# cmbant/getdist

Measured on AMD Instinct MI355X. Metric: 2D KDE densities/sec (triangle, 50 params, 1e+07 samples), higher is better.
Workload: dtype f64

## Files before the change

### getdist_amd/csrc/binning.hip

```cpp
#include "ctx.hpp"

#include <array>
#include <map>

#define LDS_HIST_BYTES (128 * 1024)

struct BinDiv {
    double binmin, width, rcp;
};
__device__ __forceinline__ BinDiv make_bindiv(double binmin, double width) {
    BinDiv d;
    d.binmin = binmin, d.width = width;
    const unsigned long long mant = (unsigned long long)__double_as_longlong(width) & 0xFFFFFFFFFFFFFull;
    d.rcp = (mant == 0xFFFFFFFFFFFFFull) ? 0.0 : 1.0 / width;
    return d;
}
__device__ __forceinline__ double bin_quotient(double x, const BinDiv& d) {
    const double n = x - d.binmin;
    double q = n * d.rcp;
    double r = fma(-q, d.width, n);
    q = fma(r, d.rcp, q);
    r = fma(-q, d.width, n);
    q = fma(r, d.rcp, q);
    if (!(fabs(q) < 1e300) || d.rcp == 0.0) q = n / d.width;
    return q;
}
__device__ __forceinline__ int bin_round(double x, const BinDiv& d) {
    return (int)(bin_quotient(x, d) + 0.5);
}
__device__ __forceinline__ int bin_trunc(double x, const BinDiv& d) {
    return (int)bin_quotient(x, d);
}

template <bool HAS_W>
__global__ void __launch_bounds__(256) k_hist1d(const double* __restrict__ cols, int64_t ld,
                                                const int32_t* __restrict__ colidx, const double* __restrict__ w,
                                                int64_t N, const double* __restrict__ binmin,
                                                const double* __restrict__ width, int F, double* __restrict__ part) {
    extern __shared__ double sh[];
    const int c = blockIdx.y;
    const double* x = cols + (int64_t)colidx[c] * ld;
    const BinDiv bd = make_bindiv(binmin[c], width[c]);
    for (int i = threadIdx.x; i < 4 * F; i += 256) sh[i] = 0;
    __syncthreads();
    double* mine = sh + (threadIdx.x >> 6) * F;
    const int64_t gtid = (int64_t)blockIdx.x * 256 + threadIdx.x, gsz = (int64_t)gridDim.x * 256;
    const int64_t Ne = N & ~(int64_t)1;
    for (int64_t i = 2 * gtid; i < Ne; i += 2 * gsz) {
        const double2 xv = *reinterpret_cast<const double2*>(x + i);
        double2 wv = make_double2(1.0, 1.0);
        if (HAS_W) wv = *reinterpret_cast<const double2*>(w + i);
        const int i0 = bin_round(xv.x, bd), i1 = bin_round(xv.y, bd);
        if ((unsigned)i0 < (unsigned)F) atomicAdd(&mine[i0], wv.x);
        if ((unsigned)i1 < (unsigned)F) atomicAdd(&mine[i1], wv.y);
    }
    if (gtid == 0 && Ne < N) {
        const int i0 = bin_round(x[Ne], bd);
        if ((unsigned)i0 < (unsigned)F) atomicAdd(&mine[i0], HAS_W ? w[Ne] : 1.0);
    }
    __syncthreads();
    double* p = part + ((int64_t)c * gridDim.x + blockIdx.x) * F;
    for (int i = threadIdx.x; i < F; i += 256) p[i] = (sh[i] + sh[F + i]) + (sh[2 * F + i] + sh[3 * F + i]);
}

__global__ void k_hist1d_reduce(const double* __restrict__ part, int nblk, int F, double* __restrict__ out) {
    const int f = blockIdx.x * blockDim.x + threadIdx.x;
    if (f >= F) return;
    const double* p = part + (int64_t)blockIdx.y * nblk * F + f;
    double s = 0;
    for (int b = 0; b < nblk; ++b) s += p[(int64_t)b * F];
    out[(int64_t)blockIdx.y * F + f] = s;
}

template <bool ROUND, typename T>
__global__ void k_bin_indices(const double* __restrict__ x, int64_t N, double binmin, double width, int F,
                              T* __restrict__ idx, unsigned long long* __restrict__ n_bad) {
    unsigned long long bad = 0;
    const BinDiv bd = make_bindiv(binmin, width);
    for (int64_t i = (int64_t)blockIdx.x * blockDim.x + threadIdx.x; i < N; i += (int64_t)gridDim.x * blockDim.x) {
        const int v = ROUND ? bin_round(x[i], bd) : bin_trunc(x[i], bd);
        idx[i] = (T)v;
        bad += ((unsigned)v >= (unsigned)F);
    }
// ... 598 lines not shown
    int64_t R = (ctx->N + nblk - 1) / nblk;
    if (R < 131072) R = 131072;
    R = (R + 4095) / 4096 * 4096;
    nblk = (int)((ctx->N + R - 1) / R);
    if (nblk < 1) nblk = 1;
    S.nblk = nblk, S.R = R, S.cap = (int)(R / 8);
    if (const char* e = getenv("GDHIP_BUCKET_LIST_CAP"))
        if (atoi(e) > 0 && atoi(e) < S.cap) S.cap = atoi(e);
    return S;
}
static int64_t bucket_route_bytes(const gd_ctx* ctx, const BucketRoute& R) {
    if (R.recs.empty()) return 0;
    const int nc = (int)R.recs.size();
    const BucketShape S = bucket_shape(ctx, nc);
    return ((int64_t)nc * sizeof(PrebinColB) + 255) / 256 * 256 + ((int64_t)nc * R.nbmax * 2 + 255) / 256 * 256 +
           ((int64_t)nc * 8 + 255) / 256 * 256 + ((int64_t)nc * S.nblk * 4 + 255) / 256 * 256 + (int64_t)nc * S.nblk * S.cap * 4 + 256;
}
template <bool OUT8>
static int bucket_route_launch(gd_ctx* ctx, const BucketRoute& R, char* base, int F, unsigned long long** bad_dev) {
    const int nc = (int)R.recs.size();
    const BucketShape S = bucket_shape(ctx, nc);
    int64_t off = 0;
    auto take = [&](int64_t bytes) {
        int64_t o = off;
        off += (bytes + 255) / 256 * 256;
        return o;
    };
    const int64_t o_recs = take((int64_t)nc * sizeof(PrebinColB)), o_lut = take((int64_t)nc * R.nbmax * 2), o_bad = take((int64_t)nc * 8),
                  o_cnt = take((int64_t)nc * S.nblk * 4), o_list = take((int64_t)nc * S.nblk * S.cap * 4);
    PrebinColB* d_recs = (PrebinColB*)(base + o_recs);
    unsigned short* d_lut = (unsigned short*)(base + o_lut);
    unsigned long long* d_bad = (unsigned long long*)(base + o_bad);
    int* d_cnt = (int*)(base + o_cnt);
    unsigned int* d_list = (unsigned int*)(base + o_list);
    GD_TRY(gd_h2d(ctx, d_recs, R.recs.data(), (size_t)nc * sizeof(PrebinColB)));
    GD_HIP(hipMemsetAsync(d_bad, 0, (size_t)nc * 8, ctx->stream));
    k_bucket_lut<<<dim3(R.nbmax / 256, nc), 256, 0, ctx->stream>>>(d_recs, F, R.nbmax, d_lut);
    GD_KERNEL_CHECK();
    const size_t lds = (size_t)R.nbmax * 2;
    GD_HIP(hipFuncSetAttribute((const void*)k_prebin_bq<OUT8>, hipFuncAttributeMaxDynamicSharedMemorySize, (int)lds));
    k_prebin_bq<OUT8><<<dim3(S.nblk, nc), 512, lds, ctx->stream>>>(d_recs, ctx->N, S.R, S.cap, R.nbmax, d_lut, d_list, d_cnt);
    GD_KERNEL_CHECK();
    k_prebin_fix<OUT8><<<dim3(S.nblk, nc), 256, 0, ctx->stream>>>(d_recs, ctx->N, S.R, S.cap, F, d_list, d_cnt, d_bad);
    GD_KERNEL_CHECK();
    *bad_dev = d_bad;
    return GD_OK;
}

#ifndef P16_UNROLL
#define P16_UNROLL 4
#endif
template <int MODE>
__global__ void __launch_bounds__(1024) k_hist2d_f64_p16(const Hist2DPair* __restrict__ pairs, int B, int64_t N, int F, int R,
                                                         int nstripes, int nchunks, int tile_major,
                                                         unsigned int* __restrict__ part, int* __restrict__ overflow) {
    extern __shared__ double sh_raw[];
    unsigned int* sh = reinterpret_cast<unsigned int*>(sh_raw);
    __shared__ double red[16];
    int pair, chunk, stripe;
    if (tile_major)
        decode_block_tiles(B, nstripes, nchunks, pair, chunk, stripe);
    else
        decode_block(nstripes, nchunks, pair, chunk, stripe);
    if (pair >= B) return;
    const Hist2DPair P = pairs[pair];
    const BinDiv bdx = make_bindiv(P.bx, P.wx), bdy = make_bindiv(P.by, P.wy);
    const int row0 = stripe * R;
    const int nwords = (R * F + 1) / 2;
    for (int i = threadIdx.x; i < nwords; i += 1024) sh[i] = 0;
    __syncthreads();
    int64_t per = (N + nchunks - 1) / nchunks;
    per = (per + 7) & ~(int64_t)7;
    const int64_t lo = (int64_t)chunk * per;
    int64_t hi = lo + per;
    if (hi > N) hi = N;
    if (hi < lo) hi = lo;
    unsigned int nacc = 0;
    auto visit = [&](double xv, double yv) {
        int cx, cy;
        if (MODE == 0) {
            cx = bin_round(xv, bdx), cy = bin_round(yv, bdy);
        } else {
            cx = bin_trunc(xv, bdx);
            cy = bin_trunc(P.r0 * xv + P.r1 * yv, bdy);
        }
        const unsigned r = (unsigned)cy - (unsigned)row0;
        if (r < (unsigned)R && (unsigned)cx < (unsigned)F && (unsigned)cy < (unsigned)F) {
            const unsigned a = r * (unsigned)F + (unsigned)cx;
            atomicAdd(&sh[a >> 1], 1u << ((a & 1u) * 16u));
            nacc += 1;
        }
    };
    const int64_t hi2 = lo + ((hi - lo) & ~(int64_t)1);
    int64_t i = lo + 2 * (int64_t)threadIdx.x;
    for (; i + (int64_t)(P16_UNROLL - 1) * 2 * 1024 < hi2; i += (int64_t)P16_UNROLL * 2 * 1024) {
        double2 xv[P16_UNROLL], yv[P16_UNROLL];
#pragma unroll
        for (int u = 0; u < P16_UNROLL; ++u) {
            xv[u] = gload_d2(P.x + i + (int64_t)u * 2 * 1024);
            yv[u] = gload_d2(P.y + i + (int64_t)u * 2 * 1024);
        }
#pragma unroll
        for (int u = 0; u < P16_UNROLL; ++u) {
            visit(xv[u].x, yv[u].x);
            visit(xv[u].y, yv[u].y);
        }
    }
    for (; i < hi2; i += 2 * 1024) {
        const double2 xv = gload_d2(P.x + i);
        const double2 yv = gload_d2(P.y + i);
        visit(xv.x, yv.x);
        visit(xv.y, yv.y);
    }
    if (threadIdx.x == 0 && hi2 < hi) visit(P.x[hi2], P.y[hi2]);
    __syncthreads();
    unsigned int* dst = part + (((int64_t)pair * nchunks + chunk) * nstripes + stripe) * (int64_t)nwords;
    unsigned int total = 0;
    for (int i = threadIdx.x; i < nwords; i += 1024) {
        const unsigned int v = sh[i];
        total += (v & 0xffffu) + (v >> 16);
        dst[i] = v;
    }
    const double t = block_sum((double)total, red), a = block_sum((double)nacc, red);
    if (threadIdx.x == 0 && t != a) atomicOr(&overflow[pair], 1);
}

__global__ void __launch_bounds__(1024) k_hist2d_u16_chunks(const Hist2DPair* __restrict__ pairs, int B, int64_t N, int F, int R,
                                                            int nstripes, int nchunks, unsigned int* __restrict__ part,
                                                            int* __restrict__ overflow) {
    extern __shared__ double sh_raw[];
    unsigned int* sh = reinterpret_cast<unsigned int*>(sh_raw);
    __shared__ double red[16];
    int pair, chunk, stripe;
    decode_block(nstripes, nchunks, pair, chunk, stripe);
    if (pair >= B) return;
    const Hist2DPair P = pairs[pair];
    const int row0 = stripe * R;
    const int nwords = (R * F + 1) / 2;
    for (int i = threadIdx.x; i < nwords; i += 1024) sh[i] = 0;
    __syncthreads();
    int64_t per = (N + nchunks - 1) / nchunks;
    per = (per + 7) & ~(int64_t)7;
    const int64_t lo = (int64_t)chunk * per;
    int64_t hi = lo + per;
    if (hi > N) hi = N;
    unsigned int nacc = 0;
    auto visit = [&](unsigned cx, unsigned cy) {
        const unsigned r = cy - (unsigned)row0;
        if (r < (unsigned)R && cx < (unsigned)F && cy < (unsigned)F) {
            const unsigned a = r * (unsigned)F + cx;
            atomicAdd(&sh[a >> 1], 1u << ((a & 1u) * 16u));
            nacc += 1;
        }
    };
    const int64_t hi8 = lo < hi ? lo + ((hi - lo) & ~(int64_t)7) : lo;
    auto visit8 = [&](const uint4& ax, const uint4& ay) {
        const unsigned xs[4] = {ax.x, ax.y, ax.z, ax.w}, ys[4] = {ay.x, ay.y, ay.z, ay.w};
#pragma unroll
        for (int q = 0; q < 4; ++q) {
            visit(xs[q] & 0xFFFFu, ys[q] & 0xFFFFu);
            visit(xs[q] >> 16, ys[q] >> 16);
        }
    };
    constexpr int DEPTH = 3;
    const int64_t nvec = (hi8 - lo) >> 3;
    const int64_t K = (nvec >> 10) / DEPTH * DEPTH;
    const uint4* gx = reinterpret_cast<const uint4*>(P.ix + lo);
    const uint4* gy = reinterpret_cast<const uint4*>(P.iy + lo);
    if (K > 0) {
        uint4 rx[DEPTH], ry[DEPTH];
#pragma unroll
        for (int d = 0; d < DEPTH; ++d) {
            rx[d] = gload_u4(gx + d * 1024 + threadIdx.x), ry[d] = gload_u4(gy + d * 1024 + threadIdx.x);
            __builtin_amdgcn_sched_barrier(0);
        }
        for (int64_t k = 0; k < K; k += DEPTH) {
            const int64_t kn = (k + DEPTH < K ? k + DEPTH : K - DEPTH) * 1024 + threadIdx.x;
#pragma unroll
            for (int d = 0; d < DEPTH; ++d) {
                visit8(rx[d], ry[d]);
                rx[d] = gload_u4(gx + kn + d * 1024), ry[d] = gload_u4(gy + kn + d * 1024);
                __builtin_amdgcn_sched_barrier(0);
            }
        }
    }
    for (int64_t u = K * 1024 + threadIdx.x; u < nvec; u += 1024) visit8(gload_u4(gx + u), gload_u4(gy + u));
    if (threadIdx.x == 0)
        for (int64_t i = hi8; i < hi; ++i) visit(P.ix[i], P.iy[i]);
    __syncthreads();
    unsigned int* dst = part + (((int64_t)pair * nchunks + chunk) * nstripes + stripe) * (int64_t)nwords;
    unsigned int total = 0;
    for (int i = threadIdx.x; i < nwords; i += 1024) {
        const unsigned int v = sh[i];
        total += (v & 0xffffu) + (v >> 16);
        dst[i] = v;
    }
    const double t = block_sum((double)total, red), a = block_sum((double)nacc, red);
    if (threadIdx.x == 0 && t != a) atomicOr(&overflow[pair], 1);
}

__global__ void __launch_bounds__(256) k_p16_reduce(const unsigned int* __restrict__ part, int F, int R, int nstripes, int nchunks,
                                                    double* __restrict__ hist_all) {
    const int pair = blockIdx.z, stripe = blockIdx.y;
    const int nwords = (R * F + 1) / 2;
    const int rows = min(R, F - stripe * R);
    const int wd = blockIdx.x * 256 + threadIdx.x;
    if (2 * wd >= rows * F) return;
    const int64_t step = (int64_t)nstripes * nwords;
    const unsigned int* p = part + ((int64_t)pair * nchunks * nstripes + stripe) * (int64_t)nwords + wd;
    unsigned int lo = 0, hi = 0;
    int c = 0;
    for (; c + 8 <= nchunks; c += 8) {
        unsigned int v[8];
#pragma unroll
        for (int q = 0; q < 8; ++q) v[q] = __builtin_nontemporal_load(p + (c + q) * step);
#pragma unroll
        for (int q = 0; q < 8; ++q) lo += v[q] & 0xffffu, hi += v[q] >> 16;
    }
    for (; c < nchunks; ++c) {
        const unsigned int v = p[c * step];
        lo += v & 0xffffu, hi += v >> 16;
    }
    double* hist = hist_all + (int64_t)pair * F * F + (int64_t)stripe * R * F;
    hist[2 * wd] = (double)lo;
    if (2 * wd + 1 < rows * F) hist[2 * wd + 1] = (double)hi;
}

__global__ void k_minmax_affine(const Hist2DPair* __restrict__ pairs, int64_t N, double* __restrict__ part) {
    __shared__ double red[16];
    const Hist2DPair P = pairs[blockIdx.y];
    double mn = INFINITY, mx = -INFINITY;
    const int64_t gtid = (int64_t)blockIdx.x * blockDim.x + threadIdx.x, gsz = (int64_t)gridDim.x * blockDim.x;
    const int64_t Ne = N & ~(int64_t)1;
    for (int64_t i = 2 * gtid; i < Ne; i += 2 * gsz) {
        const double2 xv = gload_d2(P.x + i);
        const double2 yv = gload_d2(P.y + i);
        const double p0 = P.r0 * xv.x + P.r1 * yv.x, p1 = P.r0 * xv.y + P.r1 * yv.y;
        mn = fmin(mn, fmin(p0, p1));
        mx = fmax(mx, fmax(p0, p1));
    }
    if (gtid == 0 && Ne < N) {
        const double p0 = P.r0 * P.x[Ne] + P.r1 * P.y[Ne];
        mn = fmin(mn, p0);
        mx = fmax(mx, p0);
    }
    const double r0 = block_min(mn, red), r1 = block_max(mx, red);
    if (threadIdx.x == 0) {
        double* p = part + ((int64_t)blockIdx.y * gridDim.x + blockIdx.x) * 2;
        p[0] = r0, p[1] = r1;
    }
}

#define MMG_COLS 8
#define MMG_PAIRS 16
struct MinmaxGroup {
    const double* col[MMG_COLS];
    double r0[MMG_PAIRS], r1[MMG_PAIRS];
    int a[MMG_PAIRS], b[MMG_PAIRS];
    int ncols, npairs;
};

__global__ void __launch_bounds__(256) k_minmax_affine_grouped(const MinmaxGroup* __restrict__ groups, int64_t N,
                                                               double* __restrict__ part) {
    __shared__ double2 slot[MMG_COLS][256];
    __shared__ double red[16];
    const MinmaxGroup& G = groups[blockIdx.y];
    const int ncols = G.ncols, npairs = G.npairs;
    double mn[MMG_PAIRS], mx[MMG_PAIRS];
#pragma unroll
    for (int p = 0; p < MMG_PAIRS; ++p) mn[p] = INFINITY, mx[p] = -INFINITY;
    const int64_t gtid = (int64_t)blockIdx.x * blockDim.x + threadIdx.x, gsz = (int64_t)gridDim.x * blockDim.x;
    const int64_t Ne = N & ~(int64_t)1;
    for (int64_t i = 2 * gtid; i < Ne; i += 2 * gsz) {
        double2 v[MMG_COLS];
#pragma unroll
        for (int c = 0; c < MMG_COLS; ++c) v[c] = gload_d2(G.col[min(c, ncols - 1)] + i);
        __builtin_amdgcn_sched_barrier(0);
#pragma unroll
        for (int c = 0; c < MMG_COLS; ++c) slot[c][threadIdx.x] = v[c];
#pragma unroll
        for (int p = 0; p < MMG_PAIRS; ++p)
            if (p < npairs) {
                const double2 xv = slot[G.a[p]][threadIdx.x], yv = slot[G.b[p]][threadIdx.x];
                const double p0 = G.r0[p] * xv.x + G.r1[p] * yv.x, p1 = G.r0[p] * xv.y + G.r1[p] * yv.y;
                mn[p] = fmin(mn[p], fmin(p0, p1));
                mx[p] = fmax(mx[p], fmax(p0, p1));
            }
    }
    if (gtid == 0 && Ne < N) {
#pragma unroll
        for (int p = 0; p < MMG_PAIRS; ++p)
            if (p < npairs) {
                const double p0 = G.r0[p] * G.col[G.a[p]][Ne] + G.r1[p] * G.col[G.b[p]][Ne];
                mn[p] = fmin(mn[p], p0);
                mx[p] = fmax(mx[p], p0);
            }
    }
    double* out = part + ((int64_t)blockIdx.y * gridDim.x + blockIdx.x) * MMG_PAIRS * 2;
#pragma unroll
    for (int p = 0; p < MMG_PAIRS; ++p)
        if (p < npairs) {
            const double r0 = block_min(mn[p], red), r1 = block_max(mx[p], red);
            if (threadIdx.x == 0) out[2 * p] = r0, out[2 * p + 1] = r1;
        }
}

static int pick_chunks(const gd_ctx* ctx, int64_t units, int64_t rows) {
    int best = 1;
    double best_cost = 1e30;
    for (int c = 1; c <= 16; ++c) {
        if ((int64_t)c * 65536 > rows && c > 1) break;
        const int64_t blocks = units * c;
        const double rounds = (double)((blocks + ctx->cu_count - 1) / ctx->cu_count);
        const double cost = rounds / c + 0.004 * c;
        if (cost < best_cost - 1e-12) best_cost = cost, best = c;
    }
    return best;
}

template <int MODE>
static int launch_hist2d(gd_ctx* ctx, int B, const std::vector<Hist2DPair>& hp, int F, double* d_hist, bool allow_p16 = true);

template <int MODE>
static int launch_hist2d_p16(gd_ctx* ctx, int B, const std::vector<Hist2DPair>& hp, int F, double* d_hist) {
    int R = LDS_HIST_BYTES / (F * 2);
    if (R > F) R = F;
    const int nstripes = (F + R - 1) / R;
    int nchunks = pick_chunks(ctx, (int64_t)B * nstripes, ctx->N);
    const int nwords = (R * F + 1) / 2;
    int tile_major = 0;
    if (B >= 16 && nstripes == 1 && ctx->N >= (1 << 20) && getenv("GDHIP_P16_TILE_MAJOR") != nullptr) {
        int64_t tiles = (ctx->N + 131071) / 131072;
        const int64_t cap = ((int64_t)3 << 30) / ((int64_t)B * nwords * 4);
        if (tiles > cap) tiles = cap;
        if (tiles > nchunks) nchunks = (int)tiles, tile_major = 1;
    }
    const int units = (B * nchunks + 7) / 8 * 8;
    const int64_t nblocks = (int64_t)units * nstripes;
    int64_t off = 0;
    auto take = [&](int64_t bytes) {
        int64_t o = off;
        off += (bytes + 255) / 256 * 256;
        return o;
    };
    const int64_t o_pairs = take((int64_t)B * sizeof(Hist2DPair)), o_flags = take((int64_t)B * 4),
                  o_part = take((int64_t)B * nchunks * nstripes * nwords * 4);
    char* base = (char*)gd_scratch2(ctx, off);
    if (!base) return GD_ERR_NOMEM;
    Hist2DPair* d_pairs = (Hist2DPair*)(base + o_pairs);
    int* d_flags = (int*)(base + o_flags);
    unsigned int* d_part = (unsigned int*)(base + o_part);
    GD_TRY(gd_h2d(ctx, d_pairs, hp.data(), (size_t)B * sizeof(Hist2DPair)));
    GD_HIP(hipMemsetAsync(d_flags, 0, (size_t)B * 4, ctx->stream));
    GD_HIP(hipFuncSetAttribute((const void*)k_hist2d_f64_p16<MODE>, hipFuncAttributeMaxDynamicSharedMemorySize, LDS_HIST_BYTES));
    k_hist2d_f64_p16<MODE><<<(unsigned)nblocks, 1024, (size_t)nwords * 4, ctx->stream>>>(d_pairs, B, ctx->N, F, R, nstripes,
                                                                                      nchunks, tile_major, d_part, d_flags);
    GD_KERNEL_CHECK();
    k_p16_reduce<<<dim3((unsigned)((nwords + 255) / 256), nstripes, B), 256, 0, ctx->stream>>>(d_part, F, R, nstripes, nchunks, d_hist);
    GD_KERNEL_CHECK();
    std::vector<int> hf((size_t)B);
    GD_TRY(gd_fetch(ctx, hf.data(), d_flags, (size_t)B * 4));
    GD_TRY(gd_stream_sync(ctx));
    std::vector<int> flagged;
    for (int b = 0; b < B; ++b)
        if (hf[b]) flagged.push_back(b);
    int rc = GD_OK;
    if (!flagged.empty()) {
        const int nf = (int)flagged.size();
        std::vector<Hist2DPair> sub((size_t)nf);
        for (int q = 0; q < nf; ++q) sub[q] = hp[flagged[q]];
        double* tmp = nullptr;
        GD_HIP(hipMalloc((void**)&tmp, (size_t)nf * F * F * 8));
        rc = launch_hist2d<MODE>(ctx, nf, sub, F, tmp, false);
        for (int q = 0; q < nf && rc == GD_OK; ++q)
            if (hipMemcpyAsync(d_hist + (int64_t)flagged[q] * F * F, tmp + (int64_t)q * F * F, (size_t)F * F * 8,
                               hipMemcpyDeviceToDevice, ctx->stream) != hipSuccess)
                rc = gd_fail(ctx, GD_ERR_HIP, "copy of redone histogram failed");
        (void)hipStreamSynchronize(ctx->stream);
        (void)hipFree(tmp);
    }
    return rc;
}

template <int MODE>
static int launch_hist2d(gd_ctx* ctx, int B, const std::vector<Hist2DPair>& hp, int F, double* d_hist, bool allow_p16) {
    GD_REQUIRE(F >= 2 && F <= 4096, "fine_bins_2D out of range");
    const bool has_w = ctx->w != nullptr;
    if (MODE != 2 && !has_w && allow_p16 && !getenv("GDHIP_NO_P16")) return launch_hist2d_p16<(MODE == 2 ? 0 : MODE)>(ctx, B, hp, F, d_hist);
    const bool u32bins = !has_w || ctx->w_integral;
    const int binbytes = u32bins ? 4 : 8;
    int R = LDS_HIST_BYTES / (F * binbytes);
    GD_REQUIRE(R >= 1, "fine_bins_2D too large for the LDS stripe");
    if (R > F) R = F;
    const int nstripes = (F + R - 1) / R;
    const int nchunks = pick_chunks(ctx, (int64_t)B * nstripes, ctx->N);
    const int units = (B * nchunks + 7) / 8 * 8;
    const int64_t nblocks = (int64_t)units * nstripes;
    Hist2DPair* d_pairs = (Hist2DPair*)gd_scratch2(ctx, (int64_t)B * sizeof(Hist2DPair));
    if (!d_pairs) return GD_ERR_NOMEM;
    GD_TRY(gd_h2d(ctx, d_pairs, hp.data(), (size_t)B * sizeof(Hist2DPair)));
    if (nchunks > 1) GD_HIP(hipMemsetAsync(d_hist, 0, (size_t)B * F * F * 8, ctx->stream));
    const size_t lds = (size_t)R * F * binbytes;
    if (has_w && !u32bins) {
        auto kern = k_hist2d<MODE, true, double>;
        GD_HIP(hipFuncSetAttribute((const void*)kern, hipFuncAttributeMaxDynamicSharedMemorySize, LDS_HIST_BYTES));
        kern<<<(unsigned)nblocks, 1024, lds, ctx->stream>>>(d_pairs, B, ctx->w, ctx->N, F, R, nstripes, nchunks, d_hist);
    } else if (has_w) {
        auto kern = k_hist2d<MODE, true, unsigned int>;
        GD_HIP(hipFuncSetAttribute((const void*)kern, hipFuncAttributeMaxDynamicSharedMemorySize, LDS_HIST_BYTES));
        kern<<<(unsigned)nblocks, 1024, lds, ctx->stream>>>(d_pairs, B, ctx->w, ctx->N, F, R, nstripes, nchunks, d_hist);
    } else {
        auto kern = k_hist2d<MODE, false, unsigned int>;
        GD_HIP(hipFuncSetAttribute((const void*)kern, hipFuncAttributeMaxDynamicSharedMemorySize, LDS_HIST_BYTES));
        kern<<<(unsigned)nblocks, 1024, lds, ctx->stream>>>(d_pairs, B, nullptr, ctx->N, F, R, nstripes, nchunks,
                                                            d_hist);
    }
    GD_KERNEL_CHECK();
    GD_TRY(gd_stream_sync(ctx));
    return GD_OK;
}

extern "C" {

static int hist1d_core(gd_ctx* ctx, const int32_t* cols, int32_t ncols, const double* binmin, const double* width, int32_t F,
                       double* out, bool out_on_device) {
    GD_REQUIRE(ctx && cols && binmin && width && out && ncols > 0, "bad argument");
    GD_REQUIRE(F >= 2 && F <= 4096, "fine_bins out of range (2..4096)");
    GD_REQUIRE(ctx->cols, "no samples uploaded");
    for (int i = 0; i < ncols; ++i) GD_REQUIRE(cols[i] >= 0 && cols[i] < ctx->n + GD_EXTRA_COLS, "column out of range");
    const int nblk = ctx->cu_count;
    int64_t off = 0;
    auto take = [&](int64_t bytes) {
        int64_t o = off;
        off += (bytes + 255) / 256 * 256;
        return o;
    };
    const int64_t o_part = take((int64_t)ncols * nblk * F * 8), o_out = take((int64_t)ncols * F * 8),
                  o_idx = take((int64_t)ncols * 4), o_b = take((int64_t)ncols * 8), o_w = take((int64_t)ncols * 8);
    char* base = (char*)gd_scratch(ctx, off);
    if (!base) return GD_ERR_NOMEM;
    double* d_part = (double*)(base + o_part);
    double* d_out = out_on_device ? out : (double*)(base + o_out);
    int32_t* d_idx = (int32_t*)(base + o_idx);
    double* d_b = (double*)(base + o_b);
    double* d_w = (double*)(base + o_w);
    GD_TRY(gd_h2d(ctx, d_idx, cols, (size_t)ncols * 4));
    GD_TRY(gd_h2d(ctx, d_b, binmin, (size_t)ncols * 8));
    GD_TRY(gd_h2d(ctx, d_w, width, (size_t)ncols * 8));
    dim3 grid(nblk, ncols);
    const size_t lds = (size_t)4 * F * 8;
    if (ctx->w) {
        GD_HIP(hipFuncSetAttribute((const void*)k_hist1d<true>, hipFuncAttributeMaxDynamicSharedMemorySize, 4 * 4096 * 8));
        k_hist1d<true><<<grid, 256, lds, ctx->stream>>>(ctx->cols, ctx->ld, d_idx, ctx->w, ctx->N, d_b, d_w, F, d_part);
    } else {
        GD_HIP(hipFuncSetAttribute((const void*)k_hist1d<false>, hipFuncAttributeMaxDynamicSharedMemorySize, 4 * 4096 * 8));
        k_hist1d<false><<<grid, 256, lds, ctx->stream>>>(ctx->cols, ctx->ld, d_idx, nullptr, ctx->N, d_b, d_w, F, d_part);
    }
    GD_KERNEL_CHECK();
    k_hist1d_reduce<<<dim3((F + 255) / 256, ncols), 256, 0, ctx->stream>>>(d_part, nblk, F, d_out);
    GD_KERNEL_CHECK();
    if (out_on_device) return GD_OK;
    GD_TRY(gd_fetch(ctx, out, d_out, (size_t)ncols * F * 8));
    GD_TRY(gd_stream_sync(ctx));
    return GD_OK;
}

int gd_hist1d(gd_ctx* ctx, const int32_t* cols, int32_t ncols, const double* binmin, const double* width, int32_t F,
              double* out) {
    return hist1d_core(ctx, cols, ncols, binmin, width, F, out, false);
}
int gd_hist1d_dev(gd_ctx* ctx, const int32_t* cols, int32_t ncols, const double* binmin, const double* width, int32_t F,
                  void* d_out) {
    return hist1d_core(ctx, cols, ncols, binmin, width, F, (double*)d_out, true);
}

int gd_bin_indices(gd_ctx* ctx, int32_t col, double binmin, double width, int32_t round_half, int32_t F,
                   int32_t* idx_out, int64_t* n_out_of_range) {
    GD_REQUIRE(ctx && idx_out, "bad argument");
    GD_REQUIRE(ctx->cols && col >= 0 && col < ctx->n + GD_EXTRA_COLS, "bad column");
    char* base = (char*)gd_scratch(ctx, ctx->N * 4 + 256);
    if (!base) return GD_ERR_NOMEM;
    unsigned long long* d_bad = (unsigned long long*)base;
    int32_t* d_idx = (int32_t*)(base + 256);
    GD_HIP(hipMemsetAsync(d_bad, 0, 8, ctx->stream));
    const double* x = ctx->cols + (int64_t)col * ctx->ld;
    if (round_half)
        k_bin_indices<true, int32_t><<<4 * ctx->cu_count, 256, 0, ctx->stream>>>(x, ctx->N, binmin, width, F, d_idx, d_bad);
    else
        k_bin_indices<false, int32_t><<<4 * ctx->cu_count, 256, 0, ctx->stream>>>(x, ctx->N, binmin, width, F, d_idx, d_bad);
    GD_KERNEL_CHECK();
    unsigned long long bad = 0;
    GD_TRY(gd_fetch(ctx, idx_out, d_idx, (size_t)ctx->N * 4));
    GD_TRY(gd_fetch(ctx, &bad, d_bad, 8));
    GD_TRY(gd_stream_sync(ctx));
    if (n_out_of_range) *n_out_of_range = (int64_t)bad;
    return GD_OK;
}

int gd_prebin(gd_ctx* ctx, int32_t col, double binmin, double width, int32_t F, void* d_idx_u16) {
    GD_REQUIRE(ctx && d_idx_u16, "bad argument");
    GD_REQUIRE(ctx->cols && col >= 0 && col < ctx->n + GD_EXTRA_COLS, "bad column");
    GD_REQUIRE(F >= 2 && F < 65535, "F out of range for u16 indices");
// ... 636 lines not shown
        r.idx = (unsigned char*)d_idx_out[c];
        r.binmin = binmin[c];
        r.width = width[c];
        fp_of[c] = (int)hc.size();
        hc.push_back(r);
    }
    const int nfp = (int)hc.size();
    std::vector<Hist2DPair8> hp((size_t)B);
    for (int b = 0; b < B; ++b) {
        hp[b].ix = (const unsigned char*)d_idx_x[b];
        hp[b].iy = (const unsigned char*)d_idx_y[b];
        GD_REQUIRE(hp[b].ix && hp[b].iy, "null index column");
    }
    int64_t off = 0;
    auto take = [&](int64_t bytes) {
        int64_t o = off;
        off += (bytes + 255) / 256 * 256;
        return o;
    };
    const int64_t o_cols = take((int64_t)nfp * sizeof(PrebinCol8)), o_pairs = take((int64_t)B * sizeof(Hist2DPair8));
    const int64_t table_bytes = off;
    const int64_t o_bad = take((int64_t)nfp * 8), o_flags = take((int64_t)B * 4);
    const int64_t zero_end = off;
    const int nchunks = u8_chunks(ctx, B, ctx->N);
    const int64_t o_part = take(nchunks > 1 ? (int64_t)B * nchunks * 32768 * 4 : 0);
    const int64_t o_route = take(bucket_route_bytes(ctx, R));
    char* base = (char*)gd_scratch2(ctx, off);
    if (!base) return GD_ERR_NOMEM;
    {
        std::vector<char> tab((size_t)table_bytes, 0);
        if (nfp) memcpy(tab.data() + o_cols, hc.data(), (size_t)nfp * sizeof(PrebinCol8));
        memcpy(tab.data() + o_pairs, hp.data(), (size_t)B * sizeof(Hist2DPair8));
        GD_TRY(gd_stage_h2d(ctx, base, tab.data(), (size_t)table_bytes));
    }
    GD_HIP(hipMemsetAsync(base + o_bad, 0, (size_t)(zero_end - o_bad), ctx->stream));
    if (nfp) {
        int nblk = (int)((ctx->N / 8 + 255) / 256);
        if (nblk > 2 * ctx->cu_count) nblk = 2 * ctx->cu_count;
        if (nblk < 1) nblk = 1;
        k_prebin8_batch<<<dim3(nblk, nfp), 256, 0, ctx->stream>>>((const PrebinCol8*)(base + o_cols), ctx->N, F,
                                                                 (unsigned long long*)(base + o_bad));
        GD_KERNEL_CHECK();
    }
    unsigned long long* d_bad_bq = nullptr;
    if (!R.recs.empty()) GD_TRY(bucket_route_launch<true>(ctx, R, base + o_route, F, &d_bad_bq));
    const int nblocks = (B * nchunks + 7) / 8 * 8;
    GD_HIP(hipFuncSetAttribute((const void*)k_hist2d_u8_pf<3>, hipFuncAttributeMaxDynamicSharedMemorySize, LDS_HIST_BYTES + 128));
    k_hist2d_u8_pf<3><<<nblocks, 1024, LDS_HIST_BYTES + 128, ctx->stream>>>((const Hist2DPair8*)(base + o_pairs), B, ctx->N,
                                                                            (double*)d_hist, (int*)(base + o_flags), nchunks,
                                                                            (unsigned int*)(base + o_part));
    GD_KERNEL_CHECK();
    if (nchunks > 1) {
        k_p8_reduce<<<dim3(32, B), 256, 0, ctx->stream>>>((const unsigned int*)(base + o_part), nchunks, (double*)d_hist);
        GD_KERNEL_CHECK();
    }
    std::vector<unsigned long long> hb((size_t)nfp), hq(R.recs.size());
    std::vector<int> hf((size_t)B);
    if (nfp) GD_TRY(gd_fetch(ctx, hb.data(), base + o_bad, (size_t)nfp * 8));
    if (!R.recs.empty()) GD_TRY(gd_fetch(ctx, hq.data(), d_bad_bq, hq.size() * 8));
    GD_TRY(gd_fetch(ctx, hf.data(), base + o_flags, (size_t)B * 4));
    GD_TRY(gd_stream_sync(ctx));
    int64_t nbad = 0;
    for (int c = 0; c < ncols; ++c) bad_out[c] = (int64_t)(R.slot_of[c] >= 0 ? hq[R.slot_of[c]] : hb[fp_of[c]]), nbad += bad_out[c];
    if (nbad) return gd_fail(ctx, GD_ERR_SOLVER, "%lld samples outside the byte-index grid: use the u16 path", (long long)nbad);
    for (int b = 0; b < B; ++b)
        if (hf[b]) return gd_fail(ctx, GD_ERR_SOLVER, "16-bit bin counter wrapped in pair %d: redo with gd_hist2d_prebinned", b);
    return GD_OK;
}

int gd_hist2d_sheared(gd_ctx* ctx, int32_t B, const int32_t* coli, const int32_t* colj, const double* r0,
                      const double* r1, const double* xmin, const double* dx, const double* ymin, const double* dy,
                      int32_t F, void* d_hist) {
    GD_REQUIRE(ctx && coli && colj && r0 && r1 && xmin && dx && ymin && dy && d_hist && B > 0, "bad argument");
    GD_REQUIRE(ctx->cols, "no samples uploaded");
    std::vector<Hist2DPair> hp((size_t)B);
    for (int b = 0; b < B; ++b) {
        GD_REQUIRE(coli[b] >= 0 && coli[b] < ctx->n + GD_EXTRA_COLS && colj[b] >= 0 && colj[b] < ctx->n + GD_EXTRA_COLS, "column out of range");
        Hist2DPair& p = hp[b];
        memset(&p, 0, sizeof p);
        p.x = ctx->cols + (int64_t)coli[b] * ctx->ld;
        p.y = ctx->cols + (int64_t)colj[b] * ctx->ld;
        p.bx = xmin[b], p.wx = dx[b], p.by = ymin[b], p.wy = dy[b], p.r0 = r0[b], p.r1 = r1[b];
    }
    return launch_hist2d<1>(ctx, B, hp, F, (double*)d_hist);
}

int gd_minmax_affine(gd_ctx* ctx, int32_t B, const int32_t* coli, const int32_t* colj, const double* a,
                     const double* b, double* out) {
    GD_REQUIRE(ctx && coli && colj && a && b && out && B > 0, "bad argument");
    GD_REQUIRE(ctx->cols, "no samples uploaded");
    std::vector<Hist2DPair> hp((size_t)B);
    for (int q = 0; q < B; ++q) {
        GD_REQUIRE(coli[q] >= 0 && coli[q] < ctx->n + GD_EXTRA_COLS && colj[q] >= 0 && colj[q] < ctx->n + GD_EXTRA_COLS, "column out of range");
        Hist2DPair& p = hp[q];
        memset(&p, 0, sizeof p);
        p.x = ctx->cols + (int64_t)coli[q] * ctx->ld;
        p.y = ctx->cols + (int64_t)colj[q] * ctx->ld;
        p.r0 = a[q], p.r1 = b[q];
    }
    if (B >= 4 && getenv("GDHIP_MINMAX_UNGROUPED") == nullptr) {
        std::vector<int> order((size_t)B);
        for (int q = 0; q < B; ++q) order[q] = q;
        std::sort(order.begin(), order.end(), [&](int u, int v) {
            const int ul = std::min(coli[u], colj[u]), uh = std::max(coli[u], colj[u]);
            const int vl = std::min(coli[v], colj[v]), vh = std::max(coli[v], colj[v]);
            return ul != vl ? ul < vl : (uh != vh ? uh < vh : u < v);
        });
        std::vector<MinmaxGroup> groups;
        std::vector<std::vector<int>> members;
        std::vector<int> gcols;
        auto slot_of = [&](int c) {
            for (size_t k = 0; k < gcols.size(); ++k)
                if (gcols[k] == c) return (int)k;
            return -1;
        };
        for (int q : order) {
            const int ci = coli[q], cj = colj[q];
            bool open = !groups.empty();
            if (open) {
                const int need = (slot_of(ci) < 0) + (cj != ci && slot_of(cj) < 0);
                open = (int)gcols.size() + need <= MMG_COLS && groups.back().npairs < MMG_PAIRS;
            }
            if (!open) {
                MinmaxGroup g;
                memset(&g, 0, sizeof g);
                groups.push_back(g);
                members.emplace_back();
                gcols.clear();
            }
            MinmaxGroup& g = groups.back();
            for (int c : {ci, cj})
                if (slot_of(c) < 0) {
                    g.col[gcols.size()] = ctx->cols + (int64_t)c * ctx->ld;
                    gcols.push_back(c);
                }
            g.ncols = (int)gcols.size();
            g.a[g.npairs] = slot_of(ci), g.b[g.npairs] = slot_of(cj);
            g.r0[g.npairs] = a[q], g.r1[g.npairs] = b[q];
            members.back().push_back(q);
            ++g.npairs;
        }
        const int ng = (int)groups.size();
        int nblk = (6 * ctx->cu_count + ng - 1) / ng;
        if (nblk < 8) nblk = 8;
        if (nblk > 1024) nblk = 1024;
        const int64_t o_part = ((int64_t)ng * sizeof(MinmaxGroup) + 255) / 256 * 256;
        const int64_t part_doubles = (int64_t)ng * nblk * MMG_PAIRS * 2;
        char* base = (char*)gd_scratch(ctx, o_part + part_doubles * 8);
        if (!base) return GD_ERR_NOMEM;
        GD_TRY(gd_h2d(ctx, base, groups.data(), (size_t)ng * sizeof(MinmaxGroup)));
        k_minmax_affine_grouped<<<dim3(nblk, ng), 256, 0, ctx->stream>>>((const MinmaxGroup*)base, ctx->N,
                                                                        (double*)(base + o_part));
        GD_KERNEL_CHECK();
        std::vector<double> h((size_t)part_doubles);
        GD_TRY(gd_fetch(ctx, h.data(), base + o_part, h.size() * 8));
        GD_TRY(gd_stream_sync(ctx));
        for (int g = 0; g < ng; ++g)
            for (int p = 0; p < groups[g].npairs; ++p) {
                double mn = INFINITY, mx = -INFINITY;
                for (int k = 0; k < nblk; ++k) {
                    const double* v = &h[(((size_t)g * nblk + k) * MMG_PAIRS + p) * 2];
                    if (v[0] < mn) mn = v[0];
                    if (v[1] > mx) mx = v[1];
                }
                out[2 * members[g][p]] = mn, out[2 * members[g][p] + 1] = mx;
            }
// ... 30 lines not shown
```

Before: 49730.

## Bin sheared 2D histograms from cached 16-bit bucket columns with exact fallback list

Adds a sheared-histogram path that reads precomputed 16-bit bucket indices per column instead of the f64 samples. From the bucket coordinates it decides the fine bin conservatively. Samples it cannot decide are queued in a per-wave list and re-binned exactly from the f64 data, and the whole block falls back to a full pass if the list overflows. The aim is to cut global memory traffic by about four times for most samples, at the cost of extra scratch for the lists, a host-side check of the cache records, and a dependency on bucket columns being available.

Result: faster. 50350 (median of 5 runs) (+1.2%).

```diff
diff --git a/getdist_amd/csrc/binning.hip b/getdist_amd/csrc/binning.hip
--- a/getdist_amd/csrc/binning.hip
+++ b/getdist_amd/csrc/binning.hip
@@ -1,4 +1,5 @@
 #include "ctx.hpp"
+#include "shearbucket.hpp"
 
 #include <array>
 #include <map>
@@ -763,7 +764,7 @@
             cx = bin_round(xv, bdx), cy = bin_round(yv, bdy);
         } else {
             cx = bin_trunc(xv, bdx);
-            cy = bin_trunc(P.r0 * xv + P.r1 * yv, bdy);
+            cy = bin_trunc(shear_value(P.r0, xv, P.r1, yv), bdy);
         }
         const unsigned r = (unsigned)cy - (unsigned)row0;
         if (r < (unsigned)R && (unsigned)cx < (unsigned)F && (unsigned)cy < (unsigned)F) {
@@ -907,6 +908,139 @@
     if (2 * wd + 1 < rows * F) hist[2 * wd + 1] = (double)hi;
 }
 
+struct ShearBq {
+    const unsigned short* bx;
+    const unsigned short* by;
+    ShearMap M;
+};
+#define SBQ_UNROLL 4
+#define SBQ_WAVES 16
+__global__ void __launch_bounds__(1024) k_hist2d_shear_bq(const ShearBq* __restrict__ sp, const Hist2DPair* __restrict__ pairs, int B, int64_t N,
+                                                          int F, int nchunks, int cap, unsigned int* __restrict__ lists,
+                                                          int* __restrict__ counts, unsigned int* __restrict__ part,
+                                                          int* __restrict__ overflow) {
+    extern __shared__ double sh_raw[];
+    unsigned int* sh = reinterpret_cast<unsigned int*>(sh_raw);
+    __shared__ double red[16];
+    __shared__ int wcnt[SBQ_WAVES];
+    __shared__ int over;
+    int pair, chunk, stripe;
+    decode_block(1, nchunks, pair, chunk, stripe);
+    if (pair >= B) return;
+    const ShearBq S = sp[pair];
+    const int nwords = (F * F + 1) / 2;
+    for (int i = threadIdx.x; i < nwords; i += 1024) sh[i] = 0;
+    if (threadIdx.x == 0) over = 0;
+    __syncthreads();
+    int64_t per = (N + nchunks - 1) / nchunks;
+    per = (per + 7) & ~(int64_t)7;
+    const int64_t lo = (int64_t)chunk * per;
+    int64_t hi = lo + per;
+    if (hi > N) hi = N;
+    if (hi < lo) hi = lo;
+    const int64_t nvec = (hi - lo) >> 3;
+    const unsigned short* gx = S.bx + lo;
+    const unsigned short* gy = S.by + lo;
+    const int lane = threadIdx.x & 63, wave = threadIdx.x >> 6;
+    const int capw = cap / SBQ_WAVES;
+    unsigned int* mylist = lists + ((int64_t)pair * nchunks + chunk) * cap + (int64_t)wave * capw;
+    int wcount = 0;
+    unsigned int nacc = 0;
+    auto group = [&](const uint4& ax, const uint4& ay, int64_t v, bool valid) {
+        const unsigned xs[4] = {ax.x, ax.y, ax.z, ax.w}, ys[4] = {ay.x, ay.y, ay.z, ay.w};
+        const unsigned row0 = (unsigned)(lo + 8 * v);
+#pragma unroll
+        for (int e = 0; e < 8; ++e) {
+            const unsigned bx = (e & 1) ? xs[e >> 1] >> 16 : xs[e >> 1] & 0xFFFFu, by = (e & 1) ? ys[e >> 1] >> 16 : ys[e >> 1] & 0xFFFFu;
+            const int a = sb_decide_addr(S.M, bx, by);
+            const bool hit = valid & (a >= 0), open = valid & (a < 0);
+            if (hit) atomicAdd(&sh[(unsigned)a >> 1], 1u << (((unsigned)a & 1u) * 16u));
+            nacc += hit ? 1u : 0u;
+            const unsigned long long m = __ballot(open);
+            if (open) {
+                const int pos = wcount + (int)__mbcnt_hi((unsigned)(m >> 32), __mbcnt_lo((unsigned)m, 0u));
+                if (pos < capw) mylist[pos] = row0 + (unsigned)e;
+            }
+            wcount += __popcll(m);
+        }
+    };
+    int64_t v0 = (int64_t)wave * 64;
+    for (; v0 + (int64_t)(SBQ_UNROLL - 1) * 1024 + 64 <= nvec; v0 += (int64_t)SBQ_UNROLL * 1024) {
+        const int64_t v = v0 + lane;
+        uint4 ax[SBQ_UNROLL], ay[SBQ_UNROLL];
+#pragma unroll
+        for (int u = 0; u < SBQ_UNROLL; ++u) {
+            ax[u] = gload_u4(gx + 8 * (v + u * 1024));
+            ay[u] = gload_u4(gy + 8 * (v + u * 1024));
+        }
+#pragma unroll
+        for (int u = 0; u < SBQ_UNROLL; ++u) group(ax[u], ay[u], v + u * 1024, true);
+    }
+    for (; v0 < nvec; v0 += 1024) {
+        const int64_t v = v0 + lane;
+        const bool valid = v < nvec;
+        const int64_t vl = valid ? v : nvec - 1;
+        group(gload_u4(gx + 8 * vl), gload_u4(gy + 8 * vl), v, valid);
+    }
+    if (lane == 0) {
+        wcnt[wave] = wcount;
+        if (wcount > capw) atomicOr(&over, 1);
+    }
+    __syncthreads();
+    const bool redo = over != 0;
+    const Hist2DPair P = pairs[pair];
+    const BinDiv bdx = make_bindiv(P.bx, P.wx), bdy = make_bindiv(P.by, P.wy);
+    auto visit = [&](double xv, double yv) {
+        const int cx = bin_trunc(xv, bdx);
+        const int cy = bin_trunc(shear_value(P.r0, xv, P.r1, yv), bdy);
+        if ((unsigned)cx < (unsigned)F && (unsigned)cy < (unsigned)F) {
+            const unsigned a = (unsigned)cy * (unsigned)F + (unsigned)cx;
+            atomicAdd(&sh[a >> 1], 1u << ((a & 1u) * 16u));
+            nacc += 1;
+        }
+    };
+    const int64_t hi8 = lo + 8 * nvec;
+    if (!redo) {
+        const int cnt = wcnt[wave];
+        int k = lane;
+        for (; k + 3 * 64 < cnt; k += 4 * 64) {
+            unsigned int r[4];
+#pragma unroll
+            for (int q = 0; q < 4; ++q) r[q] = mylist[k + q * 64];
+            double xv[4], yv[4];
+#pragma unroll
+            for (int q = 0; q < 4; ++q) xv[q] = P.x[r[q]], yv[q] = P.y[r[q]];
+#pragma unroll
+            for (int q = 0; q < 4; ++q) visit(xv[q], yv[q]);
+        }
+        for (; k < cnt; k += 64) {
+            const unsigned int r = mylist[k];
+            visit(P.x[r], P.y[r]);
+        }
+    } else {
+        for (int i = threadIdx.x; i < nwords; i += 1024) sh[i] = 0;
+        nacc = 0;
+        __syncthreads();
+        for (int64_t r = lo + threadIdx.x; r < hi8; r += 1024) visit(P.x[r], P.y[r]);
+    }
+    for (int64_t r = hi8 + threadIdx.x; r < hi; r += 1024) visit(P.x[r], P.y[r]);
+    __syncthreads();
+    unsigned int* dst = part + ((int64_t)pair * nchunks + chunk) * (int64_t)nwords;
+    unsigned int total = 0;
+    for (int i = threadIdx.x; i < nwords; i += 1024) {
+        const unsigned int w = sh[i];
+        total += (w & 0xffffu) + (w >> 16);
+        dst[i] = w;
+    }
+    const double t = block_sum((double)total, red), a = block_sum((double)nacc, red);
+    if (threadIdx.x == 0) {
+        int open = 0;
+        for (int w = 0; w < SBQ_WAVES; ++w) open += wcnt[w];
+        counts[(int64_t)pair * nchunks + chunk] = redo ? -1 - open : open;
+        if (t != a) atomicOr(&overflow[pair], 1);
+    }
+}
+
 __global__ void k_minmax_affine(const Hist2DPair* __restrict__ pairs, int64_t N, double* __restrict__ part) {
     __shared__ double red[16];
     const Hist2DPair P = pairs[blockIdx.y];
@@ -1001,6 +1135,8 @@
 
 template <int MODE>
 static int launch_hist2d(gd_ctx* ctx, int B, const std::vector<Hist2DPair>& hp, int F, double* d_hist, bool allow_p16 = true);
+template <int MODE>
+static int redo_flagged(gd_ctx* ctx, int B, const std::vector<Hist2DPair>& hp, const std::vector<int>& hf, int F, double* d_hist);
 
 template <int MODE>
 static int launch_hist2d_p16(gd_ctx* ctx, int B, const std::vector<Hist2DPair>& hp, int F, double* d_hist) {
@@ -1042,6 +1178,11 @@
     std::vector<int> hf((size_t)B);
     GD_TRY(gd_fetch(ctx, hf.data(), d_flags, (size_t)B * 4));
     GD_TRY(gd_stream_sync(ctx));
+    return redo_flagged<MODE>(ctx, B, hp, hf, F, d_hist);
+}
+
+template <int MODE>
+static int redo_flagged(gd_ctx* ctx, int B, const std::vector<Hist2DPair>& hp, const std::vector<int>& hf, int F, double* d_hist) {
     std::vector<int> flagged;
     for (int b = 0; b < B; ++b)
         if (hf[b]) flagged.push_back(b);
@@ -1099,6 +1240,103 @@
     GD_KERNEL_CHECK();
     GD_TRY(gd_stream_sync(ctx));
     return GD_OK;
+}
+
+struct ShearBucketRecs {
+    std::vector<SbCol> x, y;
+    std::vector<const unsigned short*> bx, by;
+};
+static bool shear_bucket_records(gd_ctx* ctx, int B, const int32_t* coli, const int32_t* colj, ShearBucketRecs* out) {
+    if (!ctx->bq) return false;
+    BucketCols& Q = *ctx->bq;
+    std::lock_guard<std::mutex> g(Q.mu);
+    if (!Q.buf || Q.ld != ctx->ld) return false;
+    out->x.resize((size_t)B), out->y.resize((size_t)B), out->bx.resize((size_t)B), out->by.resize((size_t)B);
+    for (int b = 0; b < B; ++b)
+        for (int side = 0; side < 2; ++side) {
+            const int col = side ? colj[b] : coli[b];
+            if (col < 0 || col >= Q.n || Q.nb[col] <= 0) return false;
+            SbCol r;
+            r.mn = Q.mn[col];
+            r.inv = 1.0 / Q.scale[col];
+            r.nb = Q.nb[col];
+            r.slack = sb_slack(r.mn, r.inv, r.nb);
+            if (!(r.inv > 0) || !std::isfinite(r.inv) || !std::isfinite(r.slack)) return false;
+            (side ? out->y : out->x)[b] = r;
+            (side ? out->by : out->bx)[b] = Q.buf + (int64_t)col * Q.ld;
+        }
+    return true;
+}
+static int launch_hist2d_shear_bq(gd_ctx* ctx, int B, const std::vector<Hist2DPair>& hp, const int32_t* coli, const int32_t* colj,
+                                  int F, double* d_hist, int* took) {
+    *took = 0;
+    if (ctx->w || F < 2 || F > 256 || ctx->N >= ((int64_t)1 << 32)) return GD_OK;
+    if (getenv("GDHIP_SHEAR_NO_BUCKETS") || getenv("GDHIP_NO_BUCKET_COLS") || getenv("GDHIP_NO_P16")) return GD_OK;
+    ShearBucketRecs rec;
+    if (!shear_bucket_records(ctx, B, coli, colj, &rec)) return GD_OK;
+    std::vector<ShearBq> sp((size_t)B);
+    for (int b = 0; b < B; ++b) {
+        sp[b].bx = rec.bx[b], sp[b].by = rec.by[b];
+        if (!sb_make_map(rec.x[b], rec.y[b], hp[b].bx, hp[b].wx, hp[b].by, hp[b].wy, hp[b].r0, hp[b].r1, F, &sp[b].M)) return GD_OK;
+    }
+    const int nchunks = pick_chunks(ctx, B, ctx->N);
+    const int nwords = (F * F + 1) / 2;
+    int64_t per = (ctx->N + nchunks - 1) / nchunks;
+    per = (per + 7) & ~(int64_t)7;
+    int cap = (int)(per / 8);
+    if (cap < 1) cap = 1;
+    if (const char* e = getenv("GDHIP_SHEAR_LIST_CAP"))
+        if (atoi(e) > 0 && atoi(e) < cap) cap = atoi(e);
+    const int units = (B * nchunks + 7) / 8 * 8;
+    int64_t off = 0;
+    auto take = [&](int64_t bytes) {
+        int64_t o = off;
+        off += (bytes + 255) / 256 * 256;
+        return o;
+    };
+    const int64_t o_pairs = take((int64_t)B * sizeof(Hist2DPair)), o_sp = take((int64_t)B * sizeof(ShearBq)), o_flags = take((int64_t)B * 4),
+                  o_cnt = take((int64_t)B * nchunks * 4), o_part = take((int64_t)B * nchunks * nwords * 4),
+                  o_list = take((int64_t)B * nchunks * cap * 4);
+    char* base = (char*)gd_scratch2(ctx, off);
+    if (!base) return GD_ERR_NOMEM;
+    Hist2DPair* d_pairs = (Hist2DPair*)(base + o_pairs);
+    ShearBq* d_sp = (ShearBq*)(base + o_sp);
+    int* d_flags = (int*)(base + o_flags);
+    int* d_cnt = (int*)(base + o_cnt);
+    unsigned int* d_part = (unsigned int*)(base + o_part);
+    unsigned int* d_list = (unsigned int*)(base + o_list);
+    GD_TRY(gd_h2d(ctx, d_pairs, hp.data(), (size_t)B * sizeof(Hist2DPair)));
+    GD_TRY(gd_h2d(ctx, d_sp, sp.data(), (size_t)B * sizeof(ShearBq)));
+    GD_HIP(hipMemsetAsync(d_flags, 0, (size_t)B * 4, ctx->stream));
+    GD_HIP(hipFuncSetAttribute((const void*)k_hist2d_shear_bq, hipFuncAttributeMaxDynamicSharedMemorySize, LDS_HIST_BYTES));
+    k_hist2d_shear_bq<<<(unsigned)units, 1024, (size_t)nwords * 4, ctx->stream>>>(d_sp, d_pairs, B, ctx->N, F, nchunks, cap, d_list, d_cnt, d_part,
+                                                                                 d_flags);
+    GD_KERNEL_CHECK();
+    k_p16_reduce<<<dim3((unsigned)((nwords + 255) / 256), 1, B), 256, 0, ctx->stream>>>(d_part, F, F, 1, nchunks, d_hist);
+    GD_KERNEL_CHECK();
+    std::vector<int> hf((size_t)B), hc((size_t)B * nchunks);
+    GD_TRY(gd_fetch(ctx, hf.data(), d_flags, (size_t)B * 4));
+    GD_TRY(gd_fetch(ctx, hc.data(), d_cnt, hc.size() * 4));
+    GD_TRY(gd_stream_sync(ctx));
+    {
+        ShearBucketRecs now;
+        if (!shear_bucket_records(ctx, B, coli, colj, &now)) return GD_OK;
+        auto same = [](const SbCol& a, const SbCol& b) { return a.mn == b.mn && a.inv == b.inv && a.slack == b.slack && a.nb == b.nb; };
+        for (int b = 0; b < B; ++b)
+            if (now.bx[b] != rec.bx[b] || now.by[b] != rec.by[b] || !same(now.x[b], rec.x[b]) || !same(now.y[b], rec.y[b])) return GD_OK;
+    }
+    if (getenv("GDHIP_SHEAR_STATS")) {
+        int64_t open = 0;
+        int redo = 0;
+        for (int v : hc) {
+            open += v < 0 ? -1 - v : v;
+            redo += v < 0;
+        }
+        fprintf(stderr, "gdhip shear buckets: %d pairs x %d chunks, undecided share %.5f, %d blocks redone\n", B, nchunks,
+                (double)open / ((double)B * (double)ctx->N), redo);
+    }
+    *took = 1;
+    return redo_flagged<1>(ctx, B, hp, hf, F, d_hist);
 }
 
 extern "C" {
@@ -1901,6 +2139,9 @@
         p.y = ctx->cols + (int64_t)colj[b] * ctx->ld;
         p.bx = xmin[b], p.wx = dx[b], p.by = ymin[b], p.wy = dy[b], p.r0 = r0[b], p.r1 = r1[b];
     }
+    int took = 0;
+    GD_TRY(launch_hist2d_shear_bq(ctx, B, hp, coli, colj, F, (double*)d_hist, &took));
+    if (took) return GD_OK;
     return launch_hist2d<1>(ctx, B, hp, F, (double*)d_hist);
 }
 
diff --git a/getdist_amd/csrc/shearbucket.hpp b/getdist_amd/csrc/shearbucket.hpp
--- /dev/null
+++ b/getdist_amd/csrc/shearbucket.hpp
@@ -0,0 +1,92 @@
+#pragma once
+#include <math.h>
+#include <stdint.h>
+#include <string.h>
+
+#ifndef GD_HD
+#ifdef __HIPCC__
+#define GD_HD __host__ __device__
+#else
+#define GD_HD
+#endif
+#endif
+
+#define SB_MARGIN 1.4551915228366852e-11
+
+GD_HD inline double shear_value(double r0, double x, double r1, double y) {
+    return r0 * x + r1 * y;
+}
+
+struct SbCol {
+    double mn, inv, slack;
+    int nb;
+};
+
+struct ShearMap {
+    double xa, xs, xh;
+    double va, vsx, vsy, vh;
+    double xc, vc;
+    int nbx, nby, F, pad;
+};
+
+GD_HD inline double sb_slack(double mn, double inv, int nb) {
+    const double mx = mn + (double)nb * inv;
+    return 8.0 * 2.220446049250313e-16 * fmax(fabs(mn), fabs(mx));
+}
+
+GD_HD inline bool sb_make_map(const SbCol& X, const SbCol& Y, double bx0, double wx, double by0, double wy, double r0, double r1,
+                              int F, ShearMap* out) {
+    ShearMap M;
+    if (!(wx > 0) || !(wy > 0) || !(X.inv > 0) || !(Y.inv > 0) || X.nb < 3 || Y.nb < 3 || F < 1 || F > 32768) return false;
+    const double rx = 1.0 / wx, ry = 1.0 / wy;
+    const double hx = (0.5 + 1e-3) * X.inv + X.slack, hy = (0.5 + 1e-3) * Y.inv + Y.slack;
+    const double xm = X.mn + 0.5 * X.inv, ym = Y.mn + 0.5 * Y.inv;
+    const double Mx = fmax(fabs(X.mn), fabs(X.mn + (double)X.nb * X.inv)) + X.slack;
+    const double My = fmax(fabs(Y.mn), fabs(Y.mn + (double)Y.nb * Y.inv)) + Y.slack;
+    M.xa = (xm - bx0) * rx;
+    M.xs = X.inv * rx;
+    M.xh = hx * rx + SB_MARGIN * ((Mx + fabs(bx0)) * rx + (double)F);
+    const double Mv = fabs(r0) * Mx + fabs(r1) * My;
+    M.va = ((r0 * xm + r1 * ym) - by0) * ry;
+    M.vsx = r0 * X.inv * ry;
+    M.vsy = r1 * Y.inv * ry;
+    const double allow = SB_MARGIN * (Mv + fabs(by0));
+    M.vh = ((fabs(r0) * hx + fabs(r1) * hy) + allow) * ry + SB_MARGIN * (double)F;
+    M.xc = 1.0 - 2.0 * M.xh, M.vc = 1.0 - 2.0 * M.vh;
+    M.nbx = X.nb, M.nby = Y.nb, M.F = F, M.pad = 0;
+    const double all = fabs(M.xa) + fabs(M.xs) + M.xh + fabs(M.va) + fabs(M.vsx) + fabs(M.vsy) + M.vh;
+    if (!(all < 1e300)) return false;
+    *out = M;
+    return true;
+}
+
+GD_HD inline double sb_u32_f64(unsigned b) {
+#ifdef __HIP_DEVICE_COMPILE__
+    return __hiloint2double(0x43300000, (int)b) - 4503599627370496.0;
+#else
+    const uint64_t u = 0x4330000000000000ull | (uint64_t)b;
+    double d;
+    memcpy(&d, &u, 8);
+    return d - 4503599627370496.0;
+#endif
+}
+GD_HD inline unsigned sb_f64_u32(double a) {
+    const double t = a + 4503599627370496.0;
+#ifdef __HIP_DEVICE_COMPILE__
+    return (unsigned)__double2loint(t);
+#else
+    uint64_t u;
+    memcpy(&u, &t, 8);
+    return (unsigned)u;
+#endif
+}
+GD_HD inline int sb_decide_addr(const ShearMap& M, unsigned bx, unsigned by) {
+    const double fx = sb_u32_f64(bx), fy = sb_u32_f64(by);
+    const double xl = fma(fx, M.xs, M.xa) - M.xh;
+    const double vl = fma(fx, M.vsx, fma(fy, M.vsy, M.va)) - M.vh;
+    const double kx = floor(xl), kv = floor(vl);
+    const double Fd = (double)M.F;
+    const bool ok = (xl - kx < M.xc) & (vl - kv < M.vc) & (xl > 0.0) & (xl < Fd) & (vl > 0.0) & (vl < Fd) &
+                    (bx - 1u < (unsigned)(M.nbx - 2)) & (by - 1u < (unsigned)(M.nby - 2));
+    return ok ? (int)sb_f64_u32(fma(kv, Fd, kx)) : -1;
+}
```
